# dataexplorations2026/cough_detector

Measured on AMD Instinct MI355X. Metric: 1s@16kHz clips/sec (featurise+infer), higher is better.
Workload: dtype bf16x3: split-bf16 MFMA (feature image, activations and BN-folded weights as hi+lo bf16 pairs, 3 v_mfma_f32_32x32x16_bf16 per k-step, f32 accumulate, f32 activations in HBM); featuriser f32

## Files before the change

cough_detector_amd/csrc/resblock_x3.h:

```cpp
#pragma once
#include <utility>

#include "common.h"
#include "nn_common.h"
#include "resnet_plan.h"

namespace cough {
namespace {

#ifdef COUGH_K1_STAMPS
__device__ unsigned long long* g_rb_stamp_buf = nullptr;
#define RB_STAMP(slot)                                                                        \
    do {                                                                                      \
        if (g_rb_stamp_buf && threadIdx.x == 0)                                               \
            g_rb_stamp_buf[(size_t)blockIdx.x * 8 + (slot)] = __builtin_amdgcn_s_memtime();   \
    } while (0)
#else
#define RB_STAMP(slot) do { } while (0)
#endif

struct RbxArgs {
    const float* x;
    int n_clips;
    const bf16_t* wf;
    const float* b1;
    const float* b2;
    float* out;
    const float* fcw;
    const float* fcb;
    float* logits;
    float* probs;
    int* preds;
    const int* nanflag;
};

template <int CIN, int COUT, int G, int XH, int XW>
struct RbxCfg {
    static constexpr int WAVES = 4, THREADS = 256;
    static constexpr bool T16 = rbx_t16(CIN, COUT, XH);
    static constexpr int OH = (XH - 1) / 2 + 1, OW = (XW - 1) / 2 + 1;
    static constexpr int NPX = XH * XW, PER = OH * OW, M = G * PER;
    static constexpr int NT = COUT / 32, MG = WAVES / NT, TILES = (M + 31) / 32;
    static constexpr int MW = (TILES + MG - 1) / MG;
    static constexpr int KS1 = 9 * CIN / 16, KSP = CIN / 16, KS2 = 9 * COUT / 16, KS = KS1 + KSP + KS2;
    static constexpr int CT = COUT / 16 / WAVES, NP = (M + 15) / 16;
    static constexpr int KQ1 = 9 * CIN / 32, KQP = CIN / 32, KQ2 = 9 * COUT / 32, KQ = KQ1 + KQP + KQ2;
    static_assert(!T16 || ((CT == 1 || CT == 2) && COUT == 16 * CT * WAVES && (CIN == 32 || CIN == 64) && G <= 2 &&
                           PER >= 16),
                  "T16: one or two 16-channel tiles per wave, one or two k32-steps per conv1 tap, at most one 16-pixel "
                  "tile straddling two clips");
    static constexpr int CHI = CIN / 8, CHO = COUT / 8;
    static constexpr RbxGeo L = rbx_geo(CIN, COUT, G, XH, XW);
    static_assert(L.t16 == T16 && L.m == M && L.np == NP && L.chi == CHI && L.cho == CHO, "rbx_layout describes this instantiation");
    static constexpr bool BX = L.border_x;
    static constexpr int RE = L.re, RO = L.ro;
    static constexpr int NPP = L.npp;
    static constexpr int PB01 = L.b01, PB10 = L.b10, PB11 = L.b11;
    static constexpr int NZX = BX ? rbx_x_nzero(RE, RO, OW) : 0;
    static constexpr int NPPC = L.nppc;
    static constexpr int ZC = L.zc;
    static constexpr int CPX = L.cpx;
    static constexpr int xoff(int c) { return rbx_xoff(T16, CHI, CPX, c); }
    static constexpr int ZX = L.zx;
    static constexpr int KX = L.kx;
    static constexpr int ZH = L.zh;
    static constexpr int CPH = L.cph;
    static constexpr int XBYTES = L.xbytes, HBYTES = L.hbytes;
    static_assert(!T16 || ((BX || ZX % 256 == 0) && CPX % (CHI == 4 ? 256 : 64) == 0 && CPH % 256 == 0 && (G == 1 || (NPPC - PER) % 16 == 0)),
                  "T16 bank residues");
    static_assert(!T16 || CHI == 4 || ((xoff(1) - xoff(0)) % 256 == 0 && (xoff(3) - xoff(2)) % 256 == 0 &&
                                       xoff(5) - xoff(1) == KX && xoff(6) - xoff(2) == KX && xoff(7) - xoff(3) == KX &&
                                       xoff(0) >= ZX + 256 && xoff(2) + CPX <= ZX + KX && xoff(4) >= ZX + KX + 256),
                  "T16 x layout, CIN = 64");
    static_assert(!BX || (T16 && CHI == 4 && G == 1 && XW % 2 == 1 && (16 * NP - 1 + PB11 + 1) * 16 <= CPX &&
                          PB11 + RO * OW + (RE > RO ? OW : 0) <= NPP && PB01 % 8 >= 2 && (PB11 - PB10) % 8 >= 2),
                  "bordered x planes");
    static constexpr int PL = L.pl;
    static constexpr int BIAS = L.bias;
    static constexpr int HRED = L.hred;
    static constexpr int LDS = L.lds;
    static constexpr int OP = COUT + 4;
    static_assert(T16 || (WAVES % NT == 0 && MG * MW * 32 >= M), "tile split");
    static_assert(OW == (XW + 1) / 2, "sub-image row pitch");
    static_assert(M * OP * 4 <= 2 * PL, "the output tile lies over the planes");
    static constexpr int STAGE_MAX = 18;
    static_assert((G * NPX * CIN / 4 + THREADS - 1) / THREADS <= 2 * STAGE_MAX, "staging registers (f32 input, two batches)");
    static_assert(LDS <= 160 * 1024, "one workgroup must fit a CU");
    static_assert(LDS <= 80 * 1024 || (CIN == 32 && XH > 24) || (CIN == 64 && XH == 12), "two workgroups per CU");
};

template <int CIN, int COUT, int G, int XH, int XW>
__global__ __launch_bounds__(256, 2) void resblock_x3_kernel(RbxArgs a) {
    using Cfg = RbxCfg<CIN, COUT, G, XH, XW>;
    constexpr int THREADS = Cfg::THREADS, OH = Cfg::OH, OW = Cfg::OW, NPX = Cfg::NPX, PER = Cfg::PER, M = Cfg::M;
    constexpr bool T16 = Cfg::T16;
    using f32x4 = __attribute__((ext_vector_type(4))) float;
    constexpr int CHI = Cfg::CHI, CHO = Cfg::CHO, PL = Cfg::PL, OP = Cfg::OP, CPX = Cfg::CPX, CPH = Cfg::CPH, NPP = Cfg::NPP;
    constexpr int ZX = Cfg::ZX, KX = Cfg::KX, ZH = Cfg::ZH, ZC = Cfg::ZC, NPPC = Cfg::NPPC;
#ifndef RBX_D
#define RBX_D 4
#endif
#ifndef RBX_DQ
#define RBX_DQ 3
#endif
#ifndef RBX_P
#define RBX_P 2
#endif
#ifndef RBX_PRIO
#define RBX_PRIO 0
#endif
    extern __shared__ __attribute__((aligned(256))) char smem[];
    float* lbias = reinterpret_cast<float*>(smem + Cfg::BIAS);

    const int tid = threadIdx.x, lane = tid & 63, wave = tid >> 6;
    const int clip0 = blockIdx.x * G;
    const int nvalid = a.n_clips - clip0 < G ? a.n_clips - clip0 : G;
    RB_STAMP(0);

    float bv1 = 0.f, bv2 = 0.f;
    if (tid < COUT) { bv1 = a.b1[tid]; bv2 = a.b2[tid]; }

    constexpr int CT = T16 ? Cfg::CT : 1;
    constexpr int DW = !T16 ? RBX_D : CT == 2 && G == 1 ? 2 : RBX_DQ;
    const bf16_t* wbase = a.wf + size_t(T16 ? wave * CT : wave % Cfg::NT) * 1024 + lane * 8;
    constexpr int WSTEP = T16 ? COUT / 16 : Cfg::NT;
    auto wfrag = [&](int s, int ct, int plane) -> bf16x8 {
        return *reinterpret_cast<const bf16x8*>(wbase + ((size_t(s) * WSTEP + ct) * 2 + plane) * 512);
    };
    bf16x8 ring[DW][CT][2];
#pragma unroll
    for (int i = 0; i < DW; ++i)
#pragma unroll
        for (int ct = 0; ct < CT; ++ct) { ring[i][ct][0] = wfrag(i, ct, 0); ring[i][ct][1] = wfrag(i, ct, 1); }

    {
        constexpr int NPIECE = G * NPX * CIN / 4, UN = (NPIECE + THREADS - 1) / THREADS, QP = CIN / 4;
        constexpr int NB = UN <= Cfg::STAGE_MAX ? 1 : 2, UNB = (UN + NB - 1) / NB;
        const int valid = nvalid * NPX * QP;
        const float4* src = reinterpret_cast<const float4*>(a.x + (long long)clip0 * NPX * CIN);
        if constexpr (Cfg::BX) {
            constexpr int NZX = Cfg::NZX;
            for (int z = tid; z < 2 * CHI * NZX; z += THREADS) {
                const int pl = z / NZX;
                const int cell = rbx_x_zero(Cfg::PB01, Cfg::PB10, Cfg::PB11, OW, Cfg::RE, Cfg::RO, z % NZX);
                *reinterpret_cast<uint4*>(smem + (pl / CHI) * PL + Cfg::xoff(pl % CHI) + cell * 16) = make_uint4(0, 0, 0, 0);
            }
        } else if constexpr (T16) {
            constexpr int NZ = CHI / 4;
            if (tid < 2 * NZ * ZC) {
                const int k = tid / ZC;
                *reinterpret_cast<uint4*>(smem + (k / NZ) * PL + ZX + (k % NZ) * KX + (tid % ZC) * 16) = make_uint4(0, 0, 0, 0);
            }
        } else if (tid < 2 * CHI) {
            *reinterpret_cast<uint4*>(smem + (tid / CHI) * PL + (tid % CHI) * CPX + ZX) = make_uint4(0, 0, 0, 0);
        }
#pragma unroll
        for (int b0 = 0; b0 < UN; b0 += UNB) {
            float4 v[UNB];
#pragma unroll
            for (int u = 0; u < UNB; ++u) {
                const int i = tid + (b0 + u) * THREADS;
                v[u] = src[i < valid ? i : valid - 1];
            }
#pragma unroll
            for (int u = 0; u < UNB; ++u) {
                const int i = tid + (b0 + u) * THREADS;
                if (i < NPIECE) {
                    const int P = i / QP, q = i % QP;
                    const int g = P / NPX, rem = P % NPX, ih = rem / XW, iw = rem % XW;
                    const int cell = RBX_X_CELL(g * NPPC, Cfg::PB01, Cfg::PB10, Cfg::PB11, OW, ih, iw);
                    uint2 hi, lo;
                    if (i >= valid) v[u] = make_float4(0.f, 0.f, 0.f, 0.f);
                    split4(v[u].x, v[u].y, v[u].z, v[u].w, hi, lo);
                    const int off = Cfg::xoff(q >> 1) + cell * 16 + (q & 1) * 8;
                    *reinterpret_cast<uint2*>(smem + off) = hi;
                    *reinterpret_cast<uint2*>(smem + off + PL) = lo;
                }
            }
        }
    }
    if (tid < COUT) { lbias[tid] = bv1; lbias[COUT + tid] = bv2; }
    float fw0 = 0.f, fw1 = 0.f, fb0 = 0.f, fb1 = 0.f;
    if constexpr (COUT == 128) {
        if (a.fcw != nullptr) {
            fw0 = a.fcw[tid & 127]; fw1 = a.fcw[128 + (tid & 127)];
            fb0 = a.fcb[0]; fb1 = a.fcb[1];
        }
    }
    int nan_clip = 0;
    if constexpr (COUT == 128) {
        if (a.fcw != nullptr && a.nanflag != nullptr && (tid & 127) == 0 && (tid >> 7) < nvalid) nan_clip = a.nanflag[clip0 + (tid >> 7)];
    }

    auto tapx = [](int kh, int kw) constexpr -> int { return rbx_x_tap(Cfg::PB01, Cfg::PB10, Cfg::PB11, Cfg::OW, kh, kw); };

    constexpr int NT = Cfg::NT, MW = Cfg::MW, KS1 = Cfg::KS1, KSP = Cfg::KSP, KS = Cfg::KS, D = DW;
    const int r = lane & 31, h = lane >> 5, ng = wave % NT, mg = wave / NT;
    int goh[MW], gow[MW], px1[MW], ph1[MW];
    bool rok[MW];
#pragma unroll
    for (int mt = 0; mt < MW; ++mt) {
        const int R = (mg * MW + mt) * 32 + r;
        rok[mt] = R < M;
        const int Rc = rok[mt] ? R : 0;
        const int g = Rc / PER, rem = Rc % PER;
        goh[mt] = rok[mt] ? rem / OW : -4;
        gow[mt] = rem % OW;
        px1[mt] = (g * NPP + rem) * 16 + h * CPX;
        ph1[mt] = Rc * 16 + h * CPH;
    }

    constexpr int NP = Cfg::NP, KQ1 = Cfg::KQ1, KQP = Cfg::KQP, KQ = Cfg::KQ, P = RBX_P, NB = P + 1;
    constexpr int NI = KQ * NP, I2 = (KQ1 + KQP) * NP;
    const int px = lane & 15, tq = lane >> 4, n0 = 16 * CT * wave + 4 * tq;
    unsigned vm[NP];
#pragma unroll
    for (int t = 0; t < NP; ++t) {
        const int R = 16 * t + px, rem = G > 1 ? R % PER : R, oh = rem / OW, ow = rem % OW;
        unsigned m = 0;
#pragma unroll
        for (int tap = 0; tap < 9; ++tap) {
            const int kh = tap / 3, kw = tap % 3;
            const int ih = 2 * oh - 1 + kh, iw = 2 * ow - 1 + kw, jh = oh - 1 + kh, jw = ow - 1 + kw;
            if (!Cfg::BX && unsigned(ih) < unsigned(XH) && unsigned(iw) < unsigned(XW)) m |= 1u << tap;
            if (unsigned(jh) < unsigned(OH) && unsigned(jw) < unsigned(OW)) m |= 1u << (9 + tap);
        }
        vm[t] = R < M ? m : 0u;
    }
    constexpr int DX = (NPPC - PER) * 16;
    const int lbx = px * 16 + Cfg::xoff(tq), lbh = px * 16 + tq * CPH, zh = ZH + tq * CPH;
    const int lbs = lbx + (G > 1 && px >= PER % 16 ? DX : 0);
    const int rx = px + (CHI == 4 ? 0 : Cfg::xoff(tq) / 16);
    auto zcell = [&](int z, int res) { return z + (res & 15) * 16; };
    RB_STAMP(1);
    __syncthreads();
    RB_STAMP(2);
#if RBX_PRIO
    __builtin_amdgcn_s_setprio(1);
#endif

    auto body16 = [&]() {
        f32x4 acc1[CT][NP], acc2[CT][NP];
#pragma unroll
        for (int ct = 0; ct < CT; ++ct)
#pragma unroll
            for (int t = 0; t < NP; ++t) { acc1[ct][t] = f32x4{0.f, 0.f, 0.f, 0.f}; acc2[ct][t] = f32x4{0.f, 0.f, 0.f, 0.f}; }

        int tadr[NP];
        auto aaddr = [&](auto ic) -> const char* {
            constexpr int i = decltype(ic)::value, q = i / NP, t = i % NP;
            constexpr bool conv1 = q < KQ1, proj = !conv1 && q < KQ1 + KQP;
            constexpr int kt = (conv1 ? q : proj ? q - KQ1 : q - KQ1 - KQP) * 32;
            constexpr int C = (conv1 || proj) ? CIN : COUT;
            constexpr int tap = proj ? 4 : kt / C, c32 = (kt % C) / 32, kh = tap / 3, kw = tap % 3;
            if constexpr (Cfg::BX && (conv1 || proj)) {
                return smem + lbx + (256 * t + 16 * tapx(kh, kw));
            } else if constexpr (c32 == 0) {
                if constexpr (conv1 || proj) {
                    constexpr bool strad = G > 1 && 16 * t < PER && 16 * t + 16 > PER;
                    constexpr int off = 256 * t + (G > 1 && 16 * t >= PER ? DX : 0) + 16 * tapx(kh, kw);
                    tadr[t] = (vm[t] & (1u << tap)) ? (strad ? lbs : lbx) + off : zcell(ZX, rx + tapx(kh, kw));
                } else {
                    constexpr int off = 256 * t + 16 * ((kh - 1) * OW + kw - 1);
                    tadr[t] = (vm[t] & (1u << (9 + tap))) ? lbh + off : zcell(zh, px + (kh - 1) * OW + kw - 1);
                }
            }
            return smem + tadr[t] + c32 * ((conv1 || proj) ? KX : 4 * CPH);
        };
        bf16x8 af[NB][2];
        auto fetch = [&](auto ic) {
            constexpr int i = decltype(ic)::value;
            const char* p = aaddr(ic);
            af[i % NB][0] = *reinterpret_cast<const bf16x8*>(p);
            af[i % NB][1] = *reinterpret_cast<const bf16x8*>(p + PL);
        };
        [&]<int... Js>(std::integer_sequence<int, Js...>) {
            (fetch(std::integral_constant<int, Js>{}), ...);
        }(std::make_integer_sequence<int, P>{});

        auto pair = [&]<int i>() {
            constexpr int q = i / NP, t = i % NP, j = i + P;
            if constexpr (i == I2) {
                RB_STAMP(3);
#if RBX_PRIO
                __builtin_amdgcn_s_setprio(0);
#endif
                __syncthreads();
                for (int z = tid; z < 2 * CHO * ZC; z += THREADS) {
                    const int pl = z / ZC;
                    *reinterpret_cast<uint4*>(smem + (pl / CHO) * PL + (pl % CHO) * CPH + ZH + (z % ZC) * 16) =
                        make_uint4(0, 0, 0, 0);
                }
#pragma unroll
                for (int ct = 0; ct < CT; ++ct) {
                    const int n = n0 + 16 * ct;
                    const float4 bb = *reinterpret_cast<const float4*>(lbias + n);
#pragma unroll
                    for (int u = 0; u < NP; ++u) {
                        const int R = 16 * u + px;
                        uint2 hi, lo;
                        split4(fmaxf(acc1[ct][u][0] + bb.x, 0.f), fmaxf(acc1[ct][u][1] + bb.y, 0.f),
                               fmaxf(acc1[ct][u][2] + bb.z, 0.f), fmaxf(acc1[ct][u][3] + bb.w, 0.f), hi, lo);
                        if (R < M) {
                            const int off = (n >> 3) * CPH + R * 16 + ((n >> 2) & 1) * 8;
                            *reinterpret_cast<uint2*>(smem + off) = hi;
                            *reinterpret_cast<uint2*>(smem + off + PL) = lo;
                        }
                    }
                }
                __syncthreads();
                RB_STAMP(4);
#if RBX_PRIO
                __builtin_amdgcn_s_setprio(1);
#endif
                [&]<int... Js>(std::integer_sequence<int, Js...>) {
                    (fetch(std::integral_constant<int, I2 + Js>{}), ...);
                }(std::make_integer_sequence<int, P>{});
            }
            constexpr bool pf = j < NI && (j < I2) == (i < I2);
            constexpr bool wl = t == NP - 1 && q + DW < KQ;
            const bf16x8 cur_hi = af[i % NB][0], cur_lo = af[i % NB][1];
            const char* np = nullptr;
            if constexpr (pf) np = aaddr(std::integral_constant<int, j>{});
            [&]<int... Ms>(std::integer_sequence<int, Ms...>) {
                ([&] {
                    constexpr int m = Ms, kind = m / CT, ct = m % CT;
                    const bf16x8 w = ring[q % DW][ct][kind == 2 ? 1 : 0];
                    const bf16x8 x = kind == 1 ? cur_lo : cur_hi;
                    __builtin_amdgcn_sched_barrier(0);
                    if constexpr (q < KQ1) acc1[ct][t] = __builtin_amdgcn_mfma_f32_16x16x32_bf16(w, x, acc1[ct][t], 0, 0, 0);
                    else acc2[ct][t] = __builtin_amdgcn_mfma_f32_16x16x32_bf16(w, x, acc2[ct][t], 0, 0, 0);
                    __builtin_amdgcn_sched_barrier(0);
                    if constexpr (pf && m == CT - 1) af[j % NB][0] = *reinterpret_cast<const bf16x8*>(np);
                    if constexpr (pf && m == 2 * CT - 1) af[j % NB][1] = *reinterpret_cast<const bf16x8*>(np + PL);
                    if constexpr (wl && kind == 1) ring[q % DW][ct][0] = wfrag(q + DW, ct, 0);
                    if constexpr (wl && kind == 2) ring[q % DW][ct][1] = wfrag(q + DW, ct, 1);
                }(), ...);
            }(std::make_integer_sequence<int, 3 * CT>{});
            __builtin_amdgcn_sched_barrier(0);
        };
        [&]<int... Is>(std::integer_sequence<int, Is...>) {
            (pair.template operator()<Is>(), ...);
        }(std::make_integer_sequence<int, NI>{});

        RB_STAMP(5);
#if RBX_PRIO
        __builtin_amdgcn_s_setprio(0);
#endif
        __syncthreads();
        float* otile = reinterpret_cast<float*>(smem);
#pragma unroll
        for (int ct = 0; ct < CT; ++ct) {
            const int n = n0 + 16 * ct;
            const float4 bb = *reinterpret_cast<const float4*>(lbias + COUT + n);
#pragma unroll
            for (int t = 0; t < NP; ++t) {
                const int R = 16 * t + px;
                const float4 o = make_float4(fmaxf(acc2[ct][t][0] + bb.x, 0.f), fmaxf(acc2[ct][t][1] + bb.y, 0.f),
                                             fmaxf(acc2[ct][t][2] + bb.z, 0.f), fmaxf(acc2[ct][t][3] + bb.w, 0.f));
                if (R < M) *reinterpret_cast<float4*>(otile + R * OP + n) = o;
            }
        }
    };

    auto body = [&]<int MWX>() {
        f32x16 acc1[MWX], acc2[MWX];
#pragma unroll
        for (int mt = 0; mt < MWX; ++mt) { acc1[mt] = f32x16{0}; acc2[mt] = f32x16{0}; }

        int tadr[MWX];
        auto afrag = [&](auto sc, int mt, bf16x8& fhi, bf16x8& flo) {
            constexpr int s = decltype(sc)::value;
            constexpr bool conv1 = s < KS1, proj = !conv1 && s < KS1 + KSP;
            constexpr int kt = conv1 ? s * 16 : proj ? (s - KS1) * 16 : (s - KS1 - KSP) * 16;
            constexpr int C = (conv1 || proj) ? CIN : COUT, CP = (conv1 || proj) ? CPX : CPH;
            constexpr int tap = proj ? 4 : kt / C, c16 = (kt % C) / 16, kh = tap / 3, kw = tap % 3;
            if constexpr (c16 == 0) {
                if constexpr (conv1 || proj) {
                    const int ih = 2 * goh[mt] - 1 + kh, iw = 2 * gow[mt] - 1 + kw;
                    const bool ok = unsigned(ih) < unsigned(XH) && unsigned(iw) < unsigned(XW);
                    tadr[mt] = ok ? px1[mt] + tapx(kh, kw) * 16 : ZX + h * CPX;
                } else {
                    const int ih = goh[mt] - 1 + kh, iw = gow[mt] - 1 + kw;
                    const bool ok = unsigned(ih) < unsigned(OH) && unsigned(iw) < unsigned(OW);
                    tadr[mt] = ok ? ph1[mt] + ((kh - 1) * OW + kw - 1) * 16 : ZH + h * CPH;
                }
            }
            const char* p = smem + tadr[mt] + 2 * c16 * CP;
            fhi = *reinterpret_cast<const bf16x8*>(p);
            flo = *reinterpret_cast<const bf16x8*>(p + PL);
        };
        auto aaddr = [&](auto sc, int mt) -> const char* {
            constexpr int s = decltype(sc)::value;
            constexpr bool conv1 = s < KS1, proj = !conv1 && s < KS1 + KSP;
            constexpr int kt = conv1 ? s * 16 : proj ? (s - KS1) * 16 : (s - KS1 - KSP) * 16;
            constexpr int C = (conv1 || proj) ? CIN : COUT, CP = (conv1 || proj) ? CPX : CPH;
            constexpr int tap = proj ? 4 : kt / C, c16 = (kt % C) / 16, kh = tap / 3, kw = tap % 3;
            if constexpr (c16 == 0) {
                if constexpr (conv1 || proj) {
                    const int ih = 2 * goh[mt] - 1 + kh, iw = 2 * gow[mt] - 1 + kw;
                    const bool ok = unsigned(ih) < unsigned(XH) && unsigned(iw) < unsigned(XW);
                    tadr[mt] = ok ? px1[mt] + tapx(kh, kw) * 16 : ZX + h * CPX;
                } else {
                    const int ih = goh[mt] - 1 + kh, iw = gow[mt] - 1 + kw;
                    const bool ok = unsigned(ih) < unsigned(OH) && unsigned(iw) < unsigned(OW);
                    tadr[mt] = ok ? ph1[mt] + ((kh - 1) * OW + kw - 1) * 16 : ZH + h * CPH;
                }
            }
            return smem + tadr[mt] + 2 * c16 * CP;
        };

        bf16x8 af[2][MWX][2];
#pragma unroll
        for (int mt = 0; mt < MWX; ++mt) afrag(std::integral_constant<int, 0>{}, mt, af[0][mt][0], af[0][mt][1]);

        auto step = [&]<int s>() {
            if constexpr (s == KS1 + KSP) {
                RB_STAMP(3);
#if RBX_PRIO
                __builtin_amdgcn_s_setprio(0);
#endif
                __syncthreads();
                if (tid < 2 * CHO)
                    *reinterpret_cast<uint4*>(smem + (tid / CHO) * PL + (tid % CHO) * CPH + ZH) = make_uint4(0, 0, 0, 0);
#pragma unroll
                for (int mt = 0; mt < MWX; ++mt) {
                    const int R = (mg * MW + mt) * 32 + r;
#pragma unroll
                    for (int gq = 0; gq < 4; ++gq) {
                        const int n0 = ng * 32 + 8 * gq + 4 * h;
                        const float4 bb = *reinterpret_cast<const float4*>(lbias + n0);
                        uint2 hi, lo;
                        split4(fmaxf(acc1[mt][4 * gq] + bb.x, 0.f), fmaxf(acc1[mt][4 * gq + 1] + bb.y, 0.f),
                               fmaxf(acc1[mt][4 * gq + 2] + bb.z, 0.f), fmaxf(acc1[mt][4 * gq + 3] + bb.w, 0.f), hi, lo);
                        if (rok[mt]) {
                            const int off = (n0 >> 3) * CPH + R * 16 + h * 8;
                            *reinterpret_cast<uint2*>(smem + off) = hi;
                            *reinterpret_cast<uint2*>(smem + off + PL) = lo;
                        }
                    }
                }
                __syncthreads();
                RB_STAMP(4);
#if RBX_PRIO
                __builtin_amdgcn_s_setprio(1);
#endif
#pragma unroll
                for (int mt = 0; mt < MWX; ++mt)
                    afrag(std::integral_constant<int, s>{}, mt, af[s & 1][mt][0], af[s & 1][mt][1]);
            }
            const bf16x8 whi = ring[s % D][0][0], wlo = ring[s % D][0][1];
#pragma unroll
            for (int mt = 0; mt < MWX; ++mt) {
                constexpr bool pf = s + 1 < KS && s + 1 != KS1 + KSP;
                const bf16x8 cur_hi = af[s & 1][mt][0], cur_lo = af[s & 1][mt][1];
                const char* np = nullptr;
                if constexpr (pf) np = aaddr(std::integral_constant<int, s + 1>{}, mt);
                __builtin_amdgcn_sched_barrier(0);
                if constexpr (s < KS1) acc1[mt] = __builtin_amdgcn_mfma_f32_32x32x16_bf16(whi, cur_hi, acc1[mt], 0, 0, 0);
                else acc2[mt] = __builtin_amdgcn_mfma_f32_32x32x16_bf16(whi, cur_hi, acc2[mt], 0, 0, 0);
                __builtin_amdgcn_sched_barrier(0);
                if constexpr (pf) af[(s + 1) & 1][mt][0] = *reinterpret_cast<const bf16x8*>(np);
                if constexpr (s + D < KS) { if (mt == 0) ring[s % D][0][0] = wfrag(s + D, 0, 0); }
                __builtin_amdgcn_sched_barrier(0);
                if constexpr (s < KS1) acc1[mt] = __builtin_amdgcn_mfma_f32_32x32x16_bf16(whi, cur_lo, acc1[mt], 0, 0, 0);
                else acc2[mt] = __builtin_amdgcn_mfma_f32_32x32x16_bf16(whi, cur_lo, acc2[mt], 0, 0, 0);
                __builtin_amdgcn_sched_barrier(0);
                if constexpr (pf) af[(s + 1) & 1][mt][1] = *reinterpret_cast<const bf16x8*>(np + PL);
                if constexpr (s + D < KS) { if (mt == 0) ring[s % D][0][1] = wfrag(s + D, 0, 1); }
                __builtin_amdgcn_sched_barrier(0);
                if constexpr (s < KS1) acc1[mt] = __builtin_amdgcn_mfma_f32_32x32x16_bf16(wlo, cur_hi, acc1[mt], 0, 0, 0);
                else acc2[mt] = __builtin_amdgcn_mfma_f32_32x32x16_bf16(wlo, cur_hi, acc2[mt], 0, 0, 0);
                __builtin_amdgcn_sched_barrier(0);
            }
        };
        [&]<int... Ss>(std::integer_sequence<int, Ss...>) {
            (step.template operator()<Ss>(), ...);
        }(std::make_integer_sequence<int, KS>{});

        RB_STAMP(5);
#if RBX_PRIO
        __builtin_amdgcn_s_setprio(0);
#endif
        __syncthreads();
        float* otile = reinterpret_cast<float*>(smem);
#pragma unroll
        for (int mt = 0; mt < MWX; ++mt) {
            const int R = (mg * MW + mt) * 32 + r;
#pragma unroll
            for (int gq = 0; gq < 4; ++gq) {
                const int n0 = ng * 32 + 8 * gq + 4 * h;
                const float4 bb = *reinterpret_cast<const float4*>(lbias + COUT + n0);
                const float4 o = make_float4(fmaxf(acc2[mt][4 * gq] + bb.x, 0.f), fmaxf(acc2[mt][4 * gq + 1] + bb.y, 0.f),
                                             fmaxf(acc2[mt][4 * gq + 2] + bb.z, 0.f), fmaxf(acc2[mt][4 * gq + 3] + bb.w, 0.f));
                if (rok[mt]) *reinterpret_cast<float4*>(otile + R * OP + n0) = o;
            }
        }
    };
    constexpr int TILES = Cfg::TILES;
    const int mytiles = TILES - mg * MW < MW ? TILES - mg * MW : MW;
    if constexpr (T16) {
        body16();
    } else if constexpr (MW > 1 && TILES % MW != 0) {
        if (mytiles < MW) body.template operator()<(TILES % MW)>();
        else body.template operator()<MW>();
    } else {
        body.template operator()<MW>();
    }
    __syncthreads();
    RB_STAMP(6);
    const float* otile = reinterpret_cast<const float*>(smem);
    if (a.out != nullptr) {
        const int nvec = nvalid * PER * (COUT / 4);
        float4* o = reinterpret_cast<float4*>(a.out + (long long)clip0 * PER * COUT);
        for (int p = tid; p < nvec; p += THREADS) {
            const int row = p / (COUT / 4), c4 = p % (COUT / 4);
            o[p] = *reinterpret_cast<const float4*>(otile + row * OP + 4 * c4);
        }
    }
    if constexpr (COUT == 128) {
        static_assert(G * 128 <= THREADS, "one thread per (clip, channel)");
        if (a.fcw != nullptr) {
            float* hred = reinterpret_cast<float*>(smem + Cfg::HRED);
            const int c = tid & 127, g = tid >> 7;
            float sum = 0.f;
            if (g < G) {
#pragma unroll 6
                for (int i = 0; i < PER; ++i) sum += otile[(g * PER + i) * OP + c];
            }
            const float mean = sum / float(PER);
            float l0 = wave_sum(mean * fw0), l1 = wave_sum(mean * fw1);
            if (lane == 0) { hred[wave * 2] = l0; hred[wave * 2 + 1] = l1; }
            __syncthreads();
            if (c == 0 && g < nvalid) {
                const int w0 = g * 2;
                l0 = hred[w0 * 2] + hred[(w0 + 1) * 2] + fb0;
                l1 = hred[w0 * 2 + 1] + hred[(w0 + 1) * 2 + 1] + fb1;
                const long long b = clip0 + g;
                if (nan_clip) l0 = l1 = __builtin_nanf("");
                a.logits[b * 2] = l0;
                a.logits[b * 2 + 1] = l1;
                if (a.probs) {
                    const float mx = fmaxf(l0, l1), e0 = expf(l0 - mx), e1 = expf(l1 - mx), inv = 1.0f / (e0 + e1);
                    a.probs[b * 2] = e0 * inv;
                    a.probs[b * 2 + 1] = e1 * inv;
                }
                if (a.preds) a.preds[b] = (l1 > l0) ? 1 : 0;
            }
        }
    }
    RB_STAMP(7);
}

inline void pack_x3_fragments(std::vector<bf16_t>& wf, const std::vector<float>& w1, int K1, const std::vector<float>& wp,
                              int KP, const std::vector<float>& w2, int K2, int N) {
    const int nt = N / 32, ks1 = K1 / 16, ksp = KP / 16, ks2 = K2 / 16, ks = ks1 + ksp + ks2;
    wf.assign(size_t(ks) * nt * 2 * 512, 0);
    for (int s = 0; s < ks; ++s) {
        const std::vector<float>& w = s < ks1 ? w1 : s < ks1 + ksp ? wp : w2;
        const int K = s < ks1 ? K1 : s < ks1 + ksp ? KP : K2;
        const int sl = s < ks1 ? s : s < ks1 + ksp ? s - ks1 : s - ks1 - ksp;
        for (int t = 0; t < nt; ++t)
            for (int lane = 0; lane < 64; ++lane)
                for (int jj = 0; jj < 8; ++jj) {
                    const float v = w[size_t(32 * t + (lane & 31)) * K + 16 * sl + 8 * (lane >> 5) + jj];
                    const size_t base = ((size_t(s) * nt + t) * 2) * 512 + size_t(lane) * 8 + jj;
                    split_bf16_host(v, wf[base], wf[base + 512]);
                }
    }
}

inline void pack_x3_t16_fragments(std::vector<bf16_t>& wt, const std::vector<float>& w1, int K1, const std::vector<float>& wp,
                                   int KP, const std::vector<float>& w2, int K2, int N) {
    const int nt = N / 16, q1 = K1 / 32, qp = KP / 32, q2 = K2 / 32, nq = q1 + qp + q2;
    wt.assign(size_t(nq) * nt * 2 * 512, 0);
    for (int q = 0; q < nq; ++q) {
        const std::vector<float>& w = q < q1 ? w1 : q < q1 + qp ? wp : w2;
        const int K = q < q1 ? K1 : q < q1 + qp ? KP : K2;
        const int ql = q < q1 ? q : q < q1 + qp ? q - q1 : q - q1 - qp;
        for (int t = 0; t < nt; ++t)
            for (int lane = 0; lane < 64; ++lane)
                for (int jj = 0; jj < 8; ++jj) {
                    const float v = w[size_t(16 * t + (lane & 15)) * K + 32 * ql + 8 * (lane >> 4) + jj];
                    const size_t base = ((size_t(q) * nt + t) * 2) * 512 + size_t(lane) * 8 + jj;
                    split_bf16_host(v, wt[base], wt[base + 512]);
                }
    }
}

}
}
```

Measured before the change: 6.914 million.

## Precompute tap masks at compile time and streamline address arithmetic in resblock kernel

Replaces the per-lane runtime validity bitmasks with compile-time 64-lane tap masks and selects zero-padding cells with a scalar-mask v_cndmask. Taps that are always in bounds now skip the select entirely. Weight fragments are loaded through a scalar base plus a per-lane VGPR offset with immediate offsets, and LDS fragments use 32-bit LDS address-space pointers. Input staging gets a full-tile specialisation that drops the bounds clamp. The aim is fewer VALU instructions and fewer VGPRs in the MFMA inner loop, at the cost of inline-asm constraints that may limit compiler scheduling.

```diff
diff --git a/cough_detector_amd/csrc/rbx_taps.h b/cough_detector_amd/csrc/rbx_taps.h
--- /dev/null
+++ b/cough_detector_amd/csrc/rbx_taps.h
@@ -0,0 +1,40 @@
+#pragma once
+#include "resnet_plan.h"
+
+namespace cough {
+namespace {
+
+enum RbxOperand { RBX_OP_X = 0 , RBX_OP_H = 1  };
+
+constexpr int rbx_lane_pixel(const RbxGeo L, int t, int lane) { return L.t16 ? 16 * t + (lane & 15) : 32 * t + (lane & 31); }
+
+constexpr unsigned long long rbx_tap_mask(const RbxGeo L, int op, int t, int tap) {
+    const int kh = tap / 3, kw = tap % 3;
+    unsigned long long m = 0;
+    for (int l = 0; l < 64; ++l) {
+        const int R = rbx_lane_pixel(L, t, l);
+        if (R >= L.m) continue;
+        const int rem = R % L.per, oh = rem / L.ow, ow = rem % L.ow;
+        const int ih = op == RBX_OP_X ? 2 * oh - 1 + kh : oh - 1 + kh, iw = op == RBX_OP_X ? 2 * ow - 1 + kw : ow - 1 + kw;
+        const int nh = op == RBX_OP_X ? L.xh : L.oh, nw = op == RBX_OP_X ? L.xw : L.ow;
+        if (ih >= 0 && ih < nh && iw >= 0 && iw < nw) m |= 1ull << l;
+    }
+    return m;
+}
+
+constexpr int rbx_zero_cell(int zrow, int res) { return zrow + (res & 15) * 16; }
+
+constexpr int rbx_zero_x(const RbxGeo L, int lane, int tap) {
+    if (!L.t16) return L.zx + (lane >> 5) * L.cpx;
+    const int px = lane & 15, tq = lane >> 4;
+    const int rx = px + (L.chi == 4 ? 0 : rbx_xoff(true, L.chi, L.cpx, tq) / 16);
+    return rbx_zero_cell(L.zx, rx + rbx_x_tap(L.b01, L.b10, L.b11, L.ow, tap / 3, tap % 3));
+}
+constexpr int rbx_zero_h(const RbxGeo L, int lane, int tap) {
+    if (!L.t16) return L.zh + (lane >> 5) * L.cph;
+    const int px = lane & 15, tq = lane >> 4;
+    return rbx_zero_cell(L.zh + tq * L.cph, px + rbx_h_tap(L.ow, tap / 3, tap % 3));
+}
+
+}
+}
diff --git a/cough_detector_amd/csrc/resblock_x3.h b/cough_detector_amd/csrc/resblock_x3.h
--- a/cough_detector_amd/csrc/resblock_x3.h
+++ b/cough_detector_amd/csrc/resblock_x3.h
@@ -4,6 +4,7 @@
 #include "common.h"
 #include "nn_common.h"
 #include "resnet_plan.h"
+#include "rbx_taps.h"
 
 namespace cough {
 namespace {
@@ -122,10 +123,16 @@
 
     constexpr int CT = T16 ? Cfg::CT : 1;
     constexpr int DW = !T16 ? RBX_D : CT == 2 && G == 1 ? 2 : RBX_DQ;
-    const bf16_t* wbase = a.wf + size_t(T16 ? wave * CT : wave % Cfg::NT) * 1024 + lane * 8;
+    unsigned wlane = unsigned(T16 ? wave * CT : wave % Cfg::NT) * 2048u + lane * 16u;
+#define WLANE_HERE() asm("" : "+v"(wlane))
     constexpr int WSTEP = T16 ? COUT / 16 : Cfg::NT;
+    static_assert((CT * 2 - 1) * 1024 < 4096, "channel tile and plane inside the load's immediate offset");
     auto wfrag = [&](int s, int ct, int plane) -> bf16x8 {
-        return *reinterpret_cast<const bf16x8*>(wbase + ((size_t(s) * WSTEP + ct) * 2 + plane) * 512);
+        using gbytes = const __attribute__((address_space(1))) char*;
+        using gfrag = const __attribute__((address_space(1))) bf16x8*;
+        gbytes sb = (gbytes)a.wf + size_t(s) * WSTEP * 2048;
+        asm("" : "+s"(sb));
+        return *(gfrag)(sb + wlane + (ct * 2 + plane) * 1024);
     };
     bf16x8 ring[DW][CT][2];
 #pragma unroll
@@ -136,7 +143,6 @@
     {
         constexpr int NPIECE = G * NPX * CIN / 4, UN = (NPIECE + THREADS - 1) / THREADS, QP = CIN / 4;
         constexpr int NB = UN <= Cfg::STAGE_MAX ? 1 : 2, UNB = (UN + NB - 1) / NB;
-        const int valid = nvalid * NPX * QP;
         const float4* src = reinterpret_cast<const float4*>(a.x + (long long)clip0 * NPX * CIN);
         if constexpr (Cfg::BX) {
             constexpr int NZX = Cfg::NZX;
@@ -154,30 +160,37 @@
         } else if (tid < 2 * CHI) {
             *reinterpret_cast<uint4*>(smem + (tid / CHI) * PL + (tid % CHI) * CPX + ZX) = make_uint4(0, 0, 0, 0);
         }
-#pragma unroll
-        for (int b0 = 0; b0 < UN; b0 += UNB) {
-            float4 v[UNB];
-#pragma unroll
-            for (int u = 0; u < UNB; ++u) {
-                const int i = tid + (b0 + u) * THREADS;
-                v[u] = src[i < valid ? i : valid - 1];
-            }
-#pragma unroll
-            for (int u = 0; u < UNB; ++u) {
-                const int i = tid + (b0 + u) * THREADS;
-                if (i < NPIECE) {
-                    const int P = i / QP, q = i % QP;
-                    const int g = P / NPX, rem = P % NPX, ih = rem / XW, iw = rem % XW;
-                    const int cell = RBX_X_CELL(g * NPPC, Cfg::PB01, Cfg::PB10, Cfg::PB11, OW, ih, iw);
-                    uint2 hi, lo;
-                    if (i >= valid) v[u] = make_float4(0.f, 0.f, 0.f, 0.f);
-                    split4(v[u].x, v[u].y, v[u].z, v[u].w, hi, lo);
-                    const int off = Cfg::xoff(q >> 1) + cell * 16 + (q & 1) * 8;
-                    *reinterpret_cast<uint2*>(smem + off) = hi;
-                    *reinterpret_cast<uint2*>(smem + off + PL) = lo;
-                }
-            }
-        }
+        auto stage = [&](auto fullc) {
+            constexpr bool FULL = decltype(fullc)::value;
+            const int valid = FULL ? NPIECE : nvalid * NPX * QP;
+#pragma unroll
+            for (int b0 = 0; b0 < UN; b0 += UNB) {
+                float4 v[UNB];
+#pragma unroll
+                for (int u = 0; u < UNB; ++u) {
+                    const int i = tid + (b0 + u) * THREADS;
+                    v[u] = src[i < valid ? i : valid - 1];
+                }
+#pragma unroll
+                for (int u = 0; u < UNB; ++u) {
+                    const int i = tid + (b0 + u) * THREADS;
+                    if (i < NPIECE) {
+                        const int P = i / QP, q = i % QP;
+                        const int g = P / NPX, rem = P % NPX, ih = rem / XW, iw = rem % XW;
+                        const int cell = RBX_X_CELL(g * NPPC, Cfg::PB01, Cfg::PB10, Cfg::PB11, OW, ih, iw);
+                        uint2 hi, lo;
+                        if (!FULL && i >= valid) v[u] = make_float4(0.f, 0.f, 0.f, 0.f);
+                        split4(v[u].x, v[u].y, v[u].z, v[u].w, hi, lo);
+                        const int off = Cfg::xoff(q >> 1) + cell * 16 + (q & 1) * 8;
+                        *reinterpret_cast<uint2*>(smem + off) = hi;
+                        *reinterpret_cast<uint2*>(smem + off + PL) = lo;
+                    }
+                }
+            }
+        };
+        if constexpr (G == 1) stage(std::true_type{});
+        else if (nvalid == G) stage(std::true_type{});
+        else stage(std::false_type{});
     }
     if (tid < COUT) { lbias[tid] = bv1; lbias[COUT + tid] = bv2; }
     float fw0 = 0.f, fw1 = 0.f, fb0 = 0.f, fb1 = 0.f;
@@ -213,25 +226,18 @@
     constexpr int NP = Cfg::NP, KQ1 = Cfg::KQ1, KQP = Cfg::KQP, KQ = Cfg::KQ, P = RBX_P, NB = P + 1;
     constexpr int NI = KQ * NP, I2 = (KQ1 + KQP) * NP;
     const int px = lane & 15, tq = lane >> 4, n0 = 16 * CT * wave + 4 * tq;
-    unsigned vm[NP];
-#pragma unroll
-    for (int t = 0; t < NP; ++t) {
-        const int R = 16 * t + px, rem = G > 1 ? R % PER : R, oh = rem / OW, ow = rem % OW;
-        unsigned m = 0;
-#pragma unroll
-        for (int tap = 0; tap < 9; ++tap) {
-            const int kh = tap / 3, kw = tap % 3;
-            const int ih = 2 * oh - 1 + kh, iw = 2 * ow - 1 + kw, jh = oh - 1 + kh, jw = ow - 1 + kw;
-            if (!Cfg::BX && unsigned(ih) < unsigned(XH) && unsigned(iw) < unsigned(XW)) m |= 1u << tap;
-            if (unsigned(jh) < unsigned(OH) && unsigned(jw) < unsigned(OW)) m |= 1u << (9 + tap);
-        }
-        vm[t] = R < M ? m : 0u;
-    }
+    using lds_bytes = const __attribute__((address_space(3))) char*;
+    using lds_frag = const __attribute__((address_space(3))) bf16x8*;
+    const int lds0 = int(reinterpret_cast<size_t>((lds_bytes)smem));
     constexpr int DX = (NPPC - PER) * 16;
-    const int lbx = px * 16 + Cfg::xoff(tq), lbh = px * 16 + tq * CPH, zh = ZH + tq * CPH;
+    const int lbx = lds0 + px * 16 + Cfg::xoff(tq), lbh = lds0 + px * 16 + tq * CPH, zh = lds0 + ZH + tq * CPH, zx = lds0 + ZX;
     const int lbs = lbx + (G > 1 && px >= PER % 16 ? DX : 0);
     const int rx = px + (CHI == 4 ? 0 : Cfg::xoff(tq) / 16);
-    auto zcell = [&](int z, int res) { return z + (res & 15) * 16; };
+    auto lane_select = [](unsigned long long inside, int cell, int zero) -> int {
+        int r;
+        asm("v_cndmask_b32 %0, %1, %2, %3" : "=v"(r) : "v"(zero), "v"(cell), "s"(inside));
+        return r;
+    };
     RB_STAMP(1);
     __syncthreads();
     RB_STAMP(2);
@@ -246,33 +252,55 @@
 #pragma unroll
             for (int t = 0; t < NP; ++t) { acc1[ct][t] = f32x4{0.f, 0.f, 0.f, 0.f}; acc2[ct][t] = f32x4{0.f, 0.f, 0.f, 0.f}; }
 
+        constexpr bool ZREG = !(CT == 2 && G == 1);
+        int zxc[9], zhc[9];
+        auto zero_cells = [&](auto opc) {
+            constexpr int op = decltype(opc)::value;
+            if constexpr (ZREG && !(op == RBX_OP_X && Cfg::BX)) {
+#pragma unroll
+                for (int tap = 0; tap < 9; ++tap) {
+                    int z = op == RBX_OP_X ? rbx_zero_cell(zx, rx + tapx(tap / 3, tap % 3)) : rbx_zero_cell(zh, px + rbx_h_tap(OW, tap / 3, tap % 3));
+                    asm("" : "+v"(z));
+                    (op == RBX_OP_X ? zxc : zhc)[tap] = z;
+                }
+            }
+        };
         int tadr[NP];
-        auto aaddr = [&](auto ic) -> const char* {
+        auto aaddr = [&](auto ic) -> int {
             constexpr int i = decltype(ic)::value, q = i / NP, t = i % NP;
             constexpr bool conv1 = q < KQ1, proj = !conv1 && q < KQ1 + KQP;
             constexpr int kt = (conv1 ? q : proj ? q - KQ1 : q - KQ1 - KQP) * 32;
             constexpr int C = (conv1 || proj) ? CIN : COUT;
             constexpr int tap = proj ? 4 : kt / C, c32 = (kt % C) / 32, kh = tap / 3, kw = tap % 3;
             if constexpr (Cfg::BX && (conv1 || proj)) {
-                return smem + lbx + (256 * t + 16 * tapx(kh, kw));
+                return lbx + (256 * t + 16 * tapx(kh, kw));
             } else if constexpr (c32 == 0) {
                 if constexpr (conv1 || proj) {
                     constexpr bool strad = G > 1 && 16 * t < PER && 16 * t + 16 > PER;
                     constexpr int off = 256 * t + (G > 1 && 16 * t >= PER ? DX : 0) + 16 * tapx(kh, kw);
-                    tadr[t] = (vm[t] & (1u << tap)) ? (strad ? lbs : lbx) + off : zcell(ZX, rx + tapx(kh, kw));
+                    constexpr unsigned long long in = rbx_tap_mask(Cfg::L, RBX_OP_X, t, tap);
+                    const int cell = (strad ? lbs : lbx) + off;
+                    if constexpr (in == ~0ull) tadr[t] = cell;
+                    else tadr[t] = lane_select(in, cell, ZREG ? zxc[tap] : zx | (cell & 0xF0));
                 } else {
-                    constexpr int off = 256 * t + 16 * ((kh - 1) * OW + kw - 1);
-                    tadr[t] = (vm[t] & (1u << (9 + tap))) ? lbh + off : zcell(zh, px + (kh - 1) * OW + kw - 1);
-                }
-            }
-            return smem + tadr[t] + c32 * ((conv1 || proj) ? KX : 4 * CPH);
-        };
+                    constexpr int off = 256 * t + 16 * rbx_h_tap(OW, kh, kw);
+                    constexpr unsigned long long in = rbx_tap_mask(Cfg::L, RBX_OP_H, t, tap);
+                    const int cell = lbh + off;
+                    if constexpr (in == ~0ull) tadr[t] = cell;
+                    else tadr[t] = lane_select(in, cell, ZREG ? zhc[tap] : zh | (cell & 0xF0));
+                }
+            }
+            return tadr[t] + c32 * ((conv1 || proj) ? KX : 4 * CPH);
+        };
+        auto ldsfrag = [](int addr) -> bf16x8 { return *reinterpret_cast<lds_frag>(addr); };
+        zero_cells(std::integral_constant<int, RBX_OP_X>{});
         bf16x8 af[NB][2];
+        WLANE_HERE();
         auto fetch = [&](auto ic) {
             constexpr int i = decltype(ic)::value;
-            const char* p = aaddr(ic);
-            af[i % NB][0] = *reinterpret_cast<const bf16x8*>(p);
-            af[i % NB][1] = *reinterpret_cast<const bf16x8*>(p + PL);
+            const int p = aaddr(ic);
+            af[i % NB][0] = ldsfrag(p);
+            af[i % NB][1] = ldsfrag(p + PL);
         };
         [&]<int... Js>(std::integer_sequence<int, Js...>) {
             (fetch(std::integral_constant<int, Js>{}), ...);
@@ -310,6 +338,8 @@
                 }
                 __syncthreads();
                 RB_STAMP(4);
+                WLANE_HERE();
+                zero_cells(std::integral_constant<int, RBX_OP_H>{});
 #if RBX_PRIO
                 __builtin_amdgcn_s_setprio(1);
 #endif
@@ -320,7 +350,7 @@
             constexpr bool pf = j < NI && (j < I2) == (i < I2);
             constexpr bool wl = t == NP - 1 && q + DW < KQ;
             const bf16x8 cur_hi = af[i % NB][0], cur_lo = af[i % NB][1];
-            const char* np = nullptr;
+            int np = 0;
             if constexpr (pf) np = aaddr(std::integral_constant<int, j>{});
             [&]<int... Ms>(std::integer_sequence<int, Ms...>) {
                 ([&] {
@@ -331,8 +361,8 @@
                     if constexpr (q < KQ1) acc1[ct][t] = __builtin_amdgcn_mfma_f32_16x16x32_bf16(w, x, acc1[ct][t], 0, 0, 0);
                     else acc2[ct][t] = __builtin_amdgcn_mfma_f32_16x16x32_bf16(w, x, acc2[ct][t], 0, 0, 0);
                     __builtin_amdgcn_sched_barrier(0);
-                    if constexpr (pf && m == CT - 1) af[j % NB][0] = *reinterpret_cast<const bf16x8*>(np);
-                    if constexpr (pf && m == 2 * CT - 1) af[j % NB][1] = *reinterpret_cast<const bf16x8*>(np + PL);
+                    if constexpr (pf && m == CT - 1) af[j % NB][0] = ldsfrag(np);
+                    if constexpr (pf && m == 2 * CT - 1) af[j % NB][1] = ldsfrag(np + PL);
                     if constexpr (wl && kind == 1) ring[q % DW][ct][0] = wfrag(q + DW, ct, 0);
                     if constexpr (wl && kind == 2) ring[q % DW][ct][1] = wfrag(q + DW, ct, 1);
                 }(), ...);
@@ -411,6 +441,7 @@
         };
 
         bf16x8 af[2][MWX][2];
+        WLANE_HERE();
 #pragma unroll
         for (int mt = 0; mt < MWX; ++mt) afrag(std::integral_constant<int, 0>{}, mt, af[0][mt][0], af[0][mt][1]);
 
@@ -442,6 +473,7 @@
                 }
                 __syncthreads();
                 RB_STAMP(4);
+                WLANE_HERE();
 #if RBX_PRIO
                 __builtin_amdgcn_s_setprio(1);
 #endif
@@ -551,6 +583,7 @@
     }
     RB_STAMP(7);
 }
+#undef WLANE_HERE
 
 inline void pack_x3_fragments(std::vector<bf16_t>& wf, const std::vector<float>& w1, int K1, const std::vector<float>& wp,
                               int KP, const std::vector<float>& w2, int K2, int N) {
```

Result: faster. 7.006 million, median of 6 (+1.3%).
